# 0411tony/Yue

Hardware: AMD Instinct MI355X
Metric: BPR triplet-updates/sec at k=128 (S-round semantics, user rows sequential; the reference's exact sequential semantics: secondary.exact) (higher is better)
Workload: dtype f32

## Files before the change

### yue_amd/csrc/bpr_host.hip

```cpp
#include "host_common.hpp"

#include "train_kernels.hpp"
#include "round_kernels.hpp"

using yue_host::fail;
using yue_host::kr_of;
using yue_host::with_kr;
static_assert(yue::kNllSlots == yue_host::kNllSlotsHost && yue::kHeaderSlack == yue_host::kHeaderSlackHost &&
              yue::kMetaStageMax == (uint32_t)yue_host::kMetaStageMaxHost, "host_common.hpp mirrors these");

namespace {

yue::TrainArgs make_args(yue_ctx *c, double lr, double regU, double regI) {
    yue::TrainArgs a{};
    a.P = c->P.p; a.Q = c->Q.p; a.dP = c->dP.p; a.dQ = c->dQ.p;
    a.stage = c->Q.p ? c->Q.p + (size_t)c->n * c->k : nullptr;
    a.ev_u = c->ev_u.p; a.ev_i = c->ev_i.p; a.ev_j = c->ev_j.p;
    a.indptr = c->indptr.p; a.indices = c->indices.p;
    a.nll_slots = c->scal.p;
    a.m = c->m; a.n = c->n; a.k = c->k;
    a.lr = lr;
    a.ru = (float)(lr * regU);
    a.ri = (float)(lr * regI);
    a.neg_lo = 0; a.neg_range = (int32_t)c->n;
// ... 23 lines not shown

int tpw_of(const yue_ctx *c, bool meta) { return c->opt_round_tpw ? c->opt_round_tpw : default_round_tpw(kr_of(c->k), meta); }

constexpr int64_t kMetaRangeMax = 37 * 1024;
constexpr int64_t kMetaRangesMax = 12;
constexpr int64_t kRoundGenerationsMax = 6;
constexpr double kRoundEventsPerItemRow = 4.0;

bool meta_bucketed(const yue_ctx *c) { return c->n > kMetaRangeMax * kMetaRangesMax || c->opt_round_bucket; }
bool meta_path_fits(const yue_ctx *c) { return c->opt_round_meta && c->n <= ((int64_t)yue::kBucketRangesMax << yue::kBucketShift); }

int default_round_events(yue_ctx *c, double n_rows, int64_t *out) {
    const bool fold = yue_host::fold_path(c);
    const int tpw = tpw_of(c, fold);
    int per_cu = 0, cus = 0;
    hipError_t e = hipSuccess;
    if (!with_round_instance(kr_of(c->k), tpw, [&](auto kr, auto t) {
            e = fold ? hipOccupancyMaxActiveBlocksPerMultiprocessor(&per_cu, yue::k_round_m<kr(), t()>, 256, 0)
                     : hipOccupancyMaxActiveBlocksPerMultiprocessor(&per_cu, yue::k_round<kr(), t()>, 256, 0);
        }))
        return fail(YUE_ERR_ARG, "unsupported (k, TPW) combination");
    HIPCHK(e);
    per_cu = std::min(per_cu, fold ? 7 : 6);
    HIPCHK(hipDeviceGetAttribute(&cus, hipDeviceAttributeMultiprocessorCount, c->device));
    const double slots = (double)per_cu * (double)cus;
    int64_t w = (int64_t)(slots * 4.0 * tpw);
    w -= w % 1024;
    w = std::max<int64_t>(w, 1024);
    if (fold) {
        int64_t sets = std::min<int64_t>(kRoundGenerationsMax, std::max<int64_t>(1, (int64_t)(kRoundEventsPerItemRow * n_rows / (double)w)));
        if (2.0 * (double)(w * sets) < 2.0 * n_rows) sets = std::min<int64_t>(sets, 4);
        w *= sets;
    }
    *out = w;
    return YUE_OK;
}

int launch_round(yue_ctx *c, const yue::TrainArgs &a_in, int64_t e0, int64_t e1, int64_t n0, int64_t n1,
                 int parity, int apply_p) {
    unsigned long long *cnt[2] = {c->cnt0.p, c->cnt1.p};
    uint32_t *cntp[2] = {c->cntp0.p, c->cntp1.p};
    yue::RoundArgs ra{};
    ra.e_begin = e0; ra.e_end = e1; ra.n_begin = n0; ra.n_end = n1;
    ra.cnt_cur = cnt[parity]; ra.cnt_next = cnt[parity ^ 1]; ra.cntp_cur = cntp[parity]; ra.cntp_next = cntp[parity ^ 1];
    uint32_t *tab[2] = {c->tab0.p, c->tab1.p};
    ra.tab_cur = tab[parity]; ra.tab_next = tab[parity ^ 1]; ra.staged = c->staged ? 1 : 0;
    ra.apply_p = apply_p;
// ... 24 lines not shown
int launch_round_meta(yue_ctx *c, const yue::TrainArgs &a, const std::vector<int64_t> &bounds) {
    const int64_t R = (int64_t)bounds.size() - 1;
    const int64_t E = bounds.back();
    HIPCHK(c->meta_i.resize((size_t)E + yue::kHeaderSlack)); HIPCHK(c->meta_j.resize((size_t)E + yue::kHeaderSlack));
    HIPCHK(c->round_rows.resize((size_t)R)); HIPCHK(c->d_bounds.resize((size_t)R + 1));
    if (c->h_bounds != bounds) {
        HIPCHK(hipStreamSynchronize(c->stream));
        c->h_bounds = bounds;
        HIPCHK(hipMemcpyAsync(c->d_bounds.p, c->h_bounds.data(), (size_t)(R + 1) * sizeof(int64_t), hipMemcpyHostToDevice, c->stream));
    }
    HIPCHK(hipMemsetAsync(c->round_rows.p, 0, (size_t)R * sizeof(unsigned long long), c->stream));
    HIPCHK(c->fold.resize((size_t)(E + 4 * R + 8)));
    yue::MetaArgs ma{};
    ma.ev_i = a.ev_i; ma.ev_j = a.ev_j; ma.bounds = c->d_bounds.p; ma.R = R; ma.n = (int32_t)c->n;
    const bool bucketed = meta_bucketed(c);
    if (bucketed) {
        ma.range = 1 << yue::kBucketShift;
        ma.G = (int32_t)((c->n + ma.range - 1) >> yue::kBucketShift);
        HIPCHK(c->bk_touch.resize((size_t)(2 * E + 2))); HIPCHK(c->bk_ptr.resize((size_t)R * (ma.G + 1)));
        yue::BucketArgs ba{};
        ba.ev_i = a.ev_i; ba.ev_j = a.ev_j; ba.bounds = c->d_bounds.p; ba.R = R; ba.G = ma.G;
        ba.bk_touch = c->bk_touch.p; ba.bk_ptr = c->bk_ptr.p; ba.meta_i = c->meta_i.p; ba.meta_j = c->meta_j.p;
        int cus0 = 0;
        HIPCHK(hipDeviceGetAttribute(&cus0, hipDeviceAttributeMultiprocessorCount, c->device));
        hipLaunchKernelGGL(yue::k_round_bucket, dim3((unsigned)std::min<int64_t>(R, 2 * cus0)), dim3(1024), 0, c->stream, ba);
        ma.bk_touch = c->bk_touch.p; ma.bk_ptr = c->bk_ptr.p;
    } else {
        ma.G = (int32_t)((c->n + kMetaRangeMax - 1) / kMetaRangeMax);
        ma.range = (int32_t)((c->n + ma.G - 1) / ma.G);
    }
    ma.chunk = (ma.range + 1023) / 1024; ma.chunk |= 1;
    int64_t widest = 0;
    for (int64_t r = 0; r < R; ++r) widest = std::max(widest, bounds[(size_t)r + 1] - bounds[(size_t)r]);
    const double mean_touches = 2.0 * (double)widest / (double)std::max<int64_t>(1, c->n);
    const uint32_t stage_auto = (uint32_t)std::min<double>((double)yue::kMetaStageMax, std::max<double>((double)yue::kMetaStageDefault,
                                                         std::ceil(mean_touches * (kr_of(c->k) == 1 ? 4.0 : 2.0))));
    ma.stage_max = !c->staged ? 1u : c->opt_round_stage >= 2 ? (uint32_t)c->opt_round_stage : stage_auto;
    c->last_stage_max = (int)ma.stage_max;
    ma.meta_i = c->meta_i.p; ma.meta_j = c->meta_j.p; ma.round_rows = c->round_rows.p; ma.fold = c->fold.p;
    const size_t lds = (size_t)ma.range * sizeof(uint32_t);
    const void *kfn = bucketed ? (const void *)yue::k_round_meta<true> : (const void *)yue::k_round_meta<false>;
    HIPCHK(hipFuncSetAttribute(kfn, hipFuncAttributeMaxDynamicSharedMemorySize, (int)lds));
    int per_cu = 0, cus = 0;
    if (bucketed) { HIPCHK(hipOccupancyMaxActiveBlocksPerMultiprocessor(&per_cu, yue::k_round_meta<true>, 1024, lds)); }
    else { HIPCHK(hipOccupancyMaxActiveBlocksPerMultiprocessor(&per_cu, yue::k_round_meta<false>, 1024, lds)); }
    HIPCHK(hipDeviceGetAttribute(&cus, hipDeviceAttributeMultiprocessorCount, c->device));
    const int64_t grid = std::max<int64_t>(8, std::min<int64_t>((R * ma.G + 7) / 8 * 8, (int64_t)std::max(per_cu, 1) * cus / 8 * 8));
    if (bucketed) hipLaunchKernelGGL(yue::k_round_meta<true>, dim3((unsigned)grid), dim3(1024), lds, c->stream, ma);
    else
        hipLaunchKernelGGL(yue::k_round_meta<false>, dim3((unsigned)grid), dim3(1024), lds, c->stream, ma);
    HIPCHK(hipGetLastError());
    return YUE_OK;
}

void launch_round_fold(yue_ctx *c, const yue::TrainArgs &a, int64_t e0, int64_t e1, int64_t round_index) {
    yue::FoldArgs f{};
    f.fold = c->fold.p + yue::fold_base(e0, round_index); f.round_rows = c->round_rows.p + round_index; f.Q = a.Q; f.dQ = a.dQ; f.stage = a.stage; f.k = c->k; f.capacity = (uint32_t)((e1 - e0) & ~(int64_t)3);
    const dim3 fgrid((unsigned)std::min<int64_t>(c->opt_fold_blocks, std::max<int64_t>(1, (e1 - e0 + 15) / 16))), block(256);
    with_kr(c->k, [&](auto kr) { hipLaunchKernelGGL(yue::k_round_fold<kr()>, fgrid, block, 0, c->stream, f); });
}

int launch_round_m(yue_ctx *c, const yue::TrainArgs &a_in, int64_t e0, int64_t e1, int64_t round_index) {
    yue::RoundMArgs ra{};
    ra.e_begin = e0; ra.e_end = e1; ra.staged = c->staged ? 1 : 0;
    const int tpw = tpw_of(c, true);
    const int64_t waves = (e1 - e0 + tpw - 1) / tpw;
    const int64_t blocks = (waves + 3) / 4;
    if (blocks == 0) return YUE_OK;
    const dim3 grid((unsigned)blocks), block(256);
#ifdef YUE_STAMPS
// ... 109 lines not shown
        c->ev_triplets[c->ev_used] = bounds.back() - bounds.front();
        c->ev_launches[c->ev_used] = (int64_t)ne.size();
        c->ev_used++;
    }
    return YUE_OK;
}

void reset_round_state(yue_ctx *c) {
    (void)hipStreamSynchronize(c->stream);
    if (c->cnt0.p) (void)hipMemsetAsync(c->cnt0.p, 0, c->cnt0.n * sizeof(unsigned long long), c->stream);
    if (c->cnt1.p) (void)hipMemsetAsync(c->cnt1.p, 0, c->cnt1.n * sizeof(unsigned long long), c->stream);
    if (c->cntp0.p) (void)hipMemsetAsync(c->cntp0.p, 0, c->cntp0.n * sizeof(uint32_t), c->stream);
    if (c->cntp1.p) (void)hipMemsetAsync(c->cntp1.p, 0, c->cntp1.n * sizeof(uint32_t), c->stream);
    if (c->dP.p) (void)hipMemsetAsync(c->dP.p, 0, c->dP.n * sizeof(float), c->stream);
    if (c->dQ.p) (void)hipMemsetAsync(c->dQ.p, 0, c->dQ.n * sizeof(float), c->stream);
    (void)hipStreamSynchronize(c->stream);
}

}

namespace yue_host {
bool fold_path(const yue_ctx *c) { return meta_path_fits(c); }

int zero_scalars(yue_ctx *c) {
    HIPCHK(hipMemsetAsync(c->scal.p, 0, (yue::kNllSlots + 8) * sizeof(double), c->stream));
    return YUE_OK;
}

int read_scalars(yue_ctx *c, double *nll, double *sp, double *sq) {
    double *sc = c->scal.p + yue::kNllSlots;
    hipLaunchKernelGGL(yue::k_sum_slots, dim3(1), dim3(64), 0, c->stream, c->scal.p, yue::kNllSlots, sc);
    double h[3];
    HIPCHK(hipMemcpyAsync(h, sc, sizeof h, hipMemcpyDeviceToHost, c->stream));
    HIPCHK(hipStreamSynchronize(c->stream));
    if (nll) *nll = h[0];
    if (sp) *sp = h[1];
    if (sq) *sq = h[2];
    return YUE_OK;
}

int sumsq_async(yue_ctx *c, const double *p_slots) {
    double *sc = c->scal.p + yue::kNllSlots;
    HIPCHK(hipMemsetAsync(sc + 1, 0, 2 * sizeof(double), c->stream));
    if (p_slots) hipLaunchKernelGGL(yue::k_sum_slots, dim3(1), dim3(64), 0, c->stream, p_slots, yue::kNllSlots, sc + 1);
    else hipLaunchKernelGGL(yue::k_sumsq, dim3(2048), dim3(256), 0, c->stream, c->P.p, c->m * c->k, sc + 1);
    hipLaunchKernelGGL(yue::k_sumsq, dim3(2048), dim3(256), 0, c->stream, c->Q.p, c->n * c->k, sc + 2);
// ... 3 lines not shown
int upload_triplets(yue_ctx *c, const int32_t *u, const int32_t *i, const int32_t *j, int64_t T, bool validate) {
    for (int64_t t = 0; validate && t < T; ++t) {
        if (u[t] < 0 || u[t] >= c->m || i[t] < 0 || i[t] >= c->n || j[t] >= c->n)
            return fail(YUE_ERR_ARG, "triplet " + std::to_string(t) + " out of range");
    }
    HIPCHK(c->xu.resize((size_t)T + yue::kHeaderSlack)); HIPCHK(c->xi.resize((size_t)T + yue::kHeaderSlack)); HIPCHK(c->xj.resize((size_t)T + yue::kHeaderSlack));
    HIPCHK(hipMemcpyAsync(c->xu.p, u, T * sizeof(int32_t), hipMemcpyHostToDevice, c->stream));
    HIPCHK(hipMemcpyAsync(c->xi.p, i, T * sizeof(int32_t), hipMemcpyHostToDevice, c->stream));
    HIPCHK(hipMemcpyAsync(c->xj.p, j, T * sizeof(int32_t), hipMemcpyHostToDevice, c->stream));
    return YUE_OK;
}
int adam_apply_dense(yue_ctx *c, float *var, float *m, float *v, float *grad, int64_t count, double lr, int64_t step) {
    const double b1 = 0.9, b2 = 0.999;
    const float lr_t = (float)(lr * std::sqrt(1.0 - std::pow(b2, (double)step)) / (1.0 - std::pow(b1, (double)step)));
    hipLaunchKernelGGL(yue::k_adam, dim3((unsigned)std::min<int64_t>(8192, (count + 255) / 256)), dim3(256), 0, c->stream, var, m, v, grad, count, lr_t, 0.9f, 0.999f, 1e-8f);
    HIPCHK(hipGetLastError());
    return YUE_OK;
}
int adam_apply(yue_ctx *c, double lr, int64_t step) {
    const int rc = adam_apply_dense(c, c->P.p, c->aU_m.p, c->aU_v.p, c->dP.p, c->m * (int64_t)c->k, lr, step);
    return rc ? rc : adam_apply_dense(c, c->Q.p, c->aV_m.p, c->aV_v.p, c->dQ.p, c->n * (int64_t)c->k, lr, step);
}
}
using yue_host::zero_scalars; using yue_host::read_scalars; using yue_host::sumsq_async; using yue_host::upload_triplets;

extern "C" {

int yue_bpr_replay(yue_ctx *c, const int32_t *u, const int32_t *i, const int32_t *j, int64_t T,
                   double lr, double regU, double regI, double *nll_out) {
    if (!c || !c->have_factors) return fail(YUE_ERR_ARG, "yue_bpr_replay: no factors uploaded");
    if (T < 0 || (T > 0 && (!u || !i || !j))) return fail(YUE_ERR_ARG, "yue_bpr_replay: bad triplet arrays");
    HIPCHK(hipSetDevice(c->device));
    if (!c->opt_replay_levels) {
        int rc = upload_triplets(c, u, i, j, T, false);
        if (rc) return rc;
        if ((rc = zero_scalars(c))) return rc;
        if ((rc = yue_host::chain_stream(c, T, lr, regU, regI))) return rc;
        return read_scalars(c, nll_out, nullptr, nullptr);
    }
    std::vector<int32_t> lastP((size_t)c->m, 0), lastQ((size_t)c->n, 0), lvl((size_t)T);
    int32_t nlev = 0;
    for (int64_t t = 0; t < T; ++t) {
        if (u[t] < 0 || u[t] >= c->m || i[t] < 0 || i[t] >= c->n || j[t] >= c->n) return fail(YUE_ERR_ARG, "triplet " + std::to_string(t) + " out of range");
        if (j[t] < 0) { lvl[(size_t)t] = 0; continue; }
        if (i[t] == j[t]) return fail(YUE_ERR_ARG, "triplet " + std::to_string(t) + ": i == j");
        int32_t l = std::max(lastP[(size_t)u[t]], std::max(lastQ[(size_t)i[t]], lastQ[(size_t)j[t]])) + 1;
        lvl[(size_t)t] = l;
// ... 109 lines not shown

int yue_adam_step(yue_ctx *c, const int32_t *u, const int32_t *i, const int32_t *j, int64_t T, double lr, double reg, int64_t step, double *loss_out) {
    if (!c || !c->have_factors) return fail(YUE_ERR_ARG, "yue_adam_step: no factors uploaded");
    if (T <= 0 || !u || !i || !j || step < 1) return fail(YUE_ERR_ARG, "yue_adam_step: bad argument (T > 0, step >= 1)");
    HIPCHK(hipSetDevice(c->device));
    if (c->adam_m != c->m || c->adam_n != c->n || c->adam_k != c->k) { const int rc0 = yue_adam_reset(c); if (rc0) return rc0; }
    for (int64_t t = 0; t < T; ++t)
        if (u[t] < 0 || u[t] >= c->m || i[t] < 0 || i[t] >= c->n || j[t] < 0 || j[t] >= c->n) return fail(YUE_ERR_ARG, "yue_adam_step: triplet " + std::to_string(t) + " out of range");
    int rc = upload_triplets(c, u, i, j, T, true);
    if (rc) return rc;
    if ((rc = zero_scalars(c))) return rc;
    yue::MbArgs a{};
    a.U = c->P.p; a.V = c->Q.p; a.gU = c->dP.p; a.gV = c->dQ.p; a.k = c->k; a.u = c->xu.p; a.i = c->xi.p; a.j = c->xj.p; a.T = T;
    a.reg = (float)reg; a.loss_slots = c->scal.p;
    const dim3 grid((unsigned)(((T + 31) / 32 + 3) / 4));
    with_kr(c->k, [&](auto kr) { hipLaunchKernelGGL(yue::k_mb_grad<kr()>, grid, dim3(256), 0, c->stream, a); });
    if ((rc = yue_host::adam_apply(c, lr, step))) return rc;
    return read_scalars(c, loss_out, nullptr, nullptr);
}

int yue_sample_negatives(yue_ctx *c, uint64_t seed, uint32_t epoch, int32_t *j_out) {
    if (!c || !c->have_inter || !j_out) return fail(YUE_ERR_ARG, "yue_sample_negatives: no interactions uploaded");
    HIPCHK(hipSetDevice(c->device));
    yue::TrainArgs a = make_args(c, 0, 0, 0);
    a.seed = seed; a.epoch = epoch;
    if (c->E > 0) {
        hipLaunchKernelGGL(yue::k_sample, dim3((unsigned)((c->E + 255) / 256)), dim3(256), 0, c->stream, a, c->E);
        HIPCHK(hipGetLastError());
        HIPCHK(hipMemcpyAsync(j_out, c->ev_j.p, c->E * sizeof(int32_t), hipMemcpyDeviceToHost, c->stream));
    }
    HIPCHK(hipStreamSynchronize(c->stream));
    return YUE_OK;
}

int yue_sumsq(yue_ctx *c, double *sp, double *sq) {
    if (!c || !c->have_factors) return fail(YUE_ERR_ARG, "yue_sumsq: no factors uploaded");
    HIPCHK(hipSetDevice(c->device));
    int rc = sumsq_async(c);
    if (rc) return rc;
    double h[2];
    HIPCHK(hipMemcpyAsync(h, c->scal.p + yue::kNllSlots + 1, sizeof h, hipMemcpyDeviceToHost, c->stream));
    HIPCHK(hipStreamSynchronize(c->stream));
    if (sp) *sp = h[0];
    if (sq) *sq = h[1];
    return YUE_OK;
}

int yue_bpr_epoch(yue_ctx *c, uint64_t seed, uint32_t epoch, int64_t round_events, double lr, double regU, double regI,
                  double *nll_out, double *sumsqP_out, double *sumsqQ_out) {
    if (!c || !c->have_factors || !c->have_inter) return fail(YUE_ERR_ARG, "yue_bpr_epoch: upload factors and interactions first");
    if (round_events < 0) return fail(YUE_ERR_ARG, "yue_bpr_epoch: round_events must be positive (or 0 for the device's default)");
    HIPCHK(hipSetDevice(c->device));
    yue::TrainArgs a = make_args(c, lr, regU, regI);
    a.seed = seed + 0x632BE59BD9B4E019ull * (uint64_t)c->rank;
    a.epoch = epoch;
    int rc = zero_scalars(c);
    if (rc) return rc;
    const int64_t E = c->E;
    if (E > 0) hipLaunchKernelGGL(yue::k_sample, dim3((unsigned)((E + 255) / 256)), dim3(256), 0, c->stream, a, E);
    if (c->opt_epoch_exact) {
        if (yue_host::on_communicator(c) && c->nranks > 1) return fail(YUE_ERR_ARG, "yue_bpr_epoch: option epoch_exact runs on one GPU (the sequential order spans all item shards)");
        if ((rc = yue_host::chain_epoch(c, lr, regU, regI))) return rc;
        if ((rc = sumsq_async(c))) return rc;
        return read_scalars(c, nll_out, sumsqP_out, sumsqQ_out);
    }
    std::vector<int64_t> bounds;
    double tot[2] = {(double)E, (double)c->n};
    if (yue_host::on_communicator(c)) {
        if ((rc = yue_allreduce_f64(c, tot, 2))) return rc;
        if ((rc = zero_scalars(c))) return rc;
    }
    const double etot = tot[0];
    if (round_events == 0 && (rc = default_round_events(c, tot[1] / c->nranks, &round_events))) return rc;
    int64_t ub = 1, group = 1;
    if ((rc = yue_epoch_plan(c->m, c->k, round_events, etot, c->nranks, &ub, &group, nullptr))) return rc;
    if (!yue_host::on_communicator(c)) group = std::max<int64_t>(1, (c->m + ub - 1) / ub);
    else group = std::max<int64_t>(1, ((int64_t)c->opt_comm_group_mb << 20) / std::max<int64_t>(1, ub * c->k * 4));
    std::vector<int64_t> ublock;
    for (int64_t u0 = 0; u0 < c->m; u0 += ub) { ublock.push_back(u0); bounds.push_back(c->h_ev_ptr[(size_t)u0]); }
    ublock.push_back(c->m); bounds.push_back(E);
    const int64_t R = (int64_t)ublock.size() - 1;
    const bool seq_user = !yue_host::on_communicator(c) && c->opt_round_user_seq && meta_path_fits(c);
    if (seq_user) {
        HIPCHK(c->d_ev_ptr.resize((size_t)c->m + 1));
        if (!c->d_ev_ptr_valid) {
            HIPCHK(hipMemcpyAsync(c->d_ev_ptr.p, c->h_ev_ptr.data(), ((size_t)c->m + 1) * sizeof(int64_t), hipMemcpyHostToDevice, c->stream));
            c->d_ev_ptr_valid = true;
        }
        HIPCHK(c->margins.resize((size_t)std::max<int64_t>(E, 1)));
    }
    c->psq_in_rounds = seq_user && c->all_users_have_events && E > 0;
    if (c->psq_in_rounds) {
        HIPCHK(c->psq_slots.resize((size_t)yue::kNllSlots));
        HIPCHK(hipMemsetAsync(c->psq_slots.p, 0, (size_t)yue::kNllSlots * sizeof(double), c->stream));
    }
    c->last_round_user_seq = 0;
    auto after = [&](int64_t r) -> int {
        if (seq_user && !c->bigq) { c->last_round_user_seq = 1; return YUE_OK; }
        if ((r + 1) % group != 0 && r + 1 != R) return YUE_OK;
        const int64_t g_first = ublock[(size_t)(r - (r % group))], g_last = ublock[(size_t)r + 1];
        const int64_t first = g_first * c->k, count = (g_last - g_first) * c->k;
        const dim3 grid((unsigned)std::min<int64_t>(4096, (count + 255) / 256));
        if (!yue_host::on_communicator(c)) {
            hipLaunchKernelGGL(yue::k_apply_range, grid, dim3(256), 0, c->stream, c->P.p, c->dP.p, first, count);
            return YUE_OK;
        }
        HIPCHK(hipEventRecord(c->ev_rounds, c->stream));
        HIPCHK(hipStreamWaitEvent(c->comm_stream, c->ev_rounds, 0));
        c->comm_collectives += 1;
        c->comm_bytes += (double)count * sizeof(float);
        if (const int rcr = yue_host::reduce_user_block(c, first, count, c->comm_stream)) return rcr;
        hipLaunchKernelGGL(yue::k_apply_range, grid, dim3(256), 0, c->comm_stream, c->P.p, c->dP.p, first, count);
        return YUE_OK;
// ... 88 lines not shown
```

### yue_amd/csrc/chain_host.hip

```cpp
#include "host_common.hpp"

#include <rocprim/rocprim.hpp>

#include "chain_kernels.hpp"

using yue_host::fail;
using yue_host::kr_of;

namespace {

int bits_for(uint64_t values) { int b = 1; while ((1ull << b) < values) ++b; return b; }

int rank_in_stream(yue_ctx *c, DevBuf<uint32_t> &key, DevBuf<uint32_t> &val, int64_t count, uint32_t nkeys, uint32_t *ord_a, uint32_t *ord_b) {
    if (count == 0) return YUE_OK;
    HIPCHK(c->ch_key2.resize((size_t)count)); HIPCHK(c->ch_val2.resize((size_t)count)); HIPCHK(c->ch_seg.resize((size_t)nkeys + 1));
    rocprim::double_buffer<uint32_t> dk(key.p, c->ch_key2.p), dv(val.p, c->ch_val2.p);
    size_t tmp = 0;
    const unsigned end_bit = (unsigned)bits_for((uint64_t)nkeys + 1);
    HIPCHK(rocprim::radix_sort_pairs(nullptr, tmp, dk, dv, (size_t)count, 0u, end_bit, c->stream));
    HIPCHK(c->ch_tmp.resize(tmp + 16));
    HIPCHK(rocprim::radix_sort_pairs(c->ch_tmp.p, tmp, dk, dv, (size_t)count, 0u, end_bit, c->stream));
    const dim3 grid((unsigned)((count + 255) / 256));
    hipLaunchKernelGGL(yue::k_chain_seg, grid, dim3(256), 0, c->stream, dk.current(), count, nkeys, c->ch_seg.p);
    hipLaunchKernelGGL(yue::k_chain_ord, grid, dim3(256), 0, c->stream, dk.current(), dv.current(), count, nkeys, c->ch_seg.p, ord_a, ord_b);
// ... 100 lines not shown
        unsigned long long h[8];
        HIPCHK(hipMemcpy(h, c->ch_stats.p, sizeof h, hipMemcpyDeviceToHost));
        if (split)
            fprintf(stderr, "[chain3 stats] per triplet: wave C %.0f cycles of work + %.0f waiting for a packet; wave L %.0f cycles per step without a wait (%llu steps) and %.0f waiting for room in the ring; wave S %.0f cycles waiting for packets or answers (%llu triplets)\n",
                    h[1] ? (double)h[0] / h[1] : 0.0, h[1] ? (double)h[2] / h[1] : 0.0, h[4] ? (double)h[3] / h[4] : 0.0, h[4], h[1] ? (double)h[7] / h[1] : 0.0, h[6] ? (double)h[5] / h[6] : 0.0, h[6]);
        else
        fprintf(stderr, "[chain stats] steps without a wait: %llu, %.0f cycles each; steps that waited: %llu (%.2f %%), %.0f cycles each; per run outside the steps: %.0f cycles (%llu runs)\n",
                h[1], h[1] ? (double)h[0] / h[1] : 0.0, h[3], 100.0 * h[3] / (double)(h[1] + h[3] + 1e-9), h[3] ? (double)h[2] / h[3] : 0.0, h[5] ? (double)h[4] / h[5] : 0.0, h[5]);
    }
#endif
    c->chain_runs = R; c->chain_waves = (one_xcd ? c->chain_groups : blocks) * waves_per_block;
    { float ms = 0.0f; HIPCHK(hipEventElapsedTime(&ms, c->ev_chain0, c->ev_chain1)); c->chain_kernel_us = (int64_t)(1e3 * ms); }
    if (st) return fail(YUE_ERR_HIP, std::string("exact path: a wave gave up waiting for a row (") + ((st & 2u) ? "a row's version ran past a waiting touch" : "spin limit") +
                                    "): internal error, the factors on the device are not usable");
    return YUE_OK;
}

}

namespace yue_host {

int chain_epoch(yue_ctx *c, double lr, double regU, double regI) {
    if (c->E == 0) return YUE_OK;
    HIPCHK(c->d_ev_ptr.resize((size_t)c->m + 1));
    if (!c->d_ev_ptr_valid) {
        HIPCHK(hipMemcpyAsync(c->d_ev_ptr.p, c->h_ev_ptr.data(), ((size_t)c->m + 1) * sizeof(int64_t), hipMemcpyHostToDevice, c->stream));
        c->d_ev_ptr_valid = true;
    }
    return chain_launch(c, nullptr, c->ev_i.p, c->ev_j.p, c->E, c->d_ev_ptr.p, nullptr, nullptr, c->m, lr, regU, regI);
}

int chain_stream(yue_ctx *c, int64_t T, double lr, double regU, double regI) {
    if (T == 0) return YUE_OK;
    if (T >= (1ll << 31)) return fail(YUE_ERR_ARG, "exact path: at most 2^31 - 1 triplets per call");
    HIPCHK(c->ch_head.resize((size_t)T)); HIPCHK(c->ch_incl.resize((size_t)T));
    const dim3 tgrid((unsigned)((T + 255) / 256));
    hipLaunchKernelGGL(yue::k_chain_heads, tgrid, dim3(256), 0, c->stream, c->xu.p, T, c->ch_head.p);
    size_t tmp = 0;
    HIPCHK(rocprim::inclusive_scan(nullptr, tmp, c->ch_head.p, c->ch_incl.p, (size_t)T, rocprim::plus<uint32_t>(), c->stream));
    HIPCHK(c->ch_tmp.resize(tmp + 16));
    HIPCHK(rocprim::inclusive_scan(c->ch_tmp.p, tmp, c->ch_head.p, c->ch_incl.p, (size_t)T, rocprim::plus<uint32_t>(), c->stream));
    uint32_t R32 = 0;
    HIPCHK(hipMemcpyAsync(&R32, c->ch_incl.p + (T - 1), sizeof R32, hipMemcpyDeviceToHost, c->stream));
    HIPCHK(hipStreamSynchronize(c->stream));
    const int64_t R = R32;
    HIPCHK(c->ch_run_ptr.resize((size_t)R + 1)); HIPCHK(c->ch_run_u.resize((size_t)R)); HIPCHK(c->ch_ord_u.resize((size_t)R));
    HIPCHK(c->ch_rkey.resize((size_t)R)); HIPCHK(c->ch_rval.resize((size_t)R));
    hipLaunchKernelGGL(yue::k_chain_runs, tgrid, dim3(256), 0, c->stream, c->xu.p, c->ch_head.p, c->ch_incl.p, T, c->ch_run_ptr.p, c->ch_run_u.p, c->ch_rkey.p, c->ch_rval.p, (uint32_t)c->m);
    int rc = rank_in_stream(c, c->ch_rkey, c->ch_rval, R, (uint32_t)c->m, c->ch_ord_u.p, nullptr);
    if (rc) return rc;
    return chain_launch(c, c->xu.p, c->xi.p, c->xj.p, T, c->ch_run_ptr.p, c->ch_run_u.p, c->ch_ord_u.p, R, lr, regU, regI);
// ... 4 lines not shown
```

### yue_amd/csrc/core_host.hip

```cpp
#include "host_common.hpp"

namespace yue_host {
thread_local std::string g_err;
int fail(int code, const std::string &msg) { g_err = msg; return code; }
}
using yue_host::fail;
void yue_comm_release(yue_ctx *c);

extern "C" {

const char *yue_last_error(void) { return yue_host::g_err.c_str(); }
int yue_version(void) { return 1; }

int yue_ctx_create(int device, yue_ctx **out) {
    if (!out) return fail(YUE_ERR_ARG, "yue_ctx_create: out is NULL");
    int ndev = 0;
    HIPCHK(hipGetDeviceCount(&ndev));
    if (ndev <= 0) return fail(YUE_ERR_HIP, "no HIP device visible: libyue_hip needs an MI355X (no CPU fallback exists)");
    if (device < 0 || device >= ndev) return fail(YUE_ERR_ARG, "device ordinal out of range");
    HIPCHK(hipSetDevice(device));
    yue_ctx *c = new yue_ctx();
    c->device = device;
    const auto init = [c]() -> int {
        HIPCHK(hipStreamCreateWithFlags(&c->stream, hipStreamNonBlocking));
// ... 109 lines not shown
        if (indptr[u + 1] < indptr[u] || ev_ptr[u + 1] < ev_ptr[u]) return fail(YUE_ERR_ARG, "yue_set_interactions: offsets must be non-decreasing");
        for (int64_t t = indptr[u]; t < indptr[u + 1]; ++t) {
            if (indices[t] < 0 || indices[t] >= n) return fail(YUE_ERR_ARG, "yue_set_interactions: item id out of range");
            if (t > indptr[u] && indices[t] <= indices[t - 1]) return fail(YUE_ERR_ARG, "yue_set_interactions: rows must be sorted and unique");
        }
        if (indptr[u + 1] - indptr[u] >= n) return fail(YUE_ERR_ARG, "yue_set_interactions: a user listened to every item (the reference's sampler would never return, BPR.py:47)");
    }
    const int64_t nnz = indptr[m], E = ev_ptr[m];
    {
        int64_t prev = -1, max_gap = 0;
        for (int64_t u = 0; u < m; ++u) if (ev_ptr[u + 1] > ev_ptr[u]) { if (prev >= 0) max_gap = std::max(max_gap, u - prev); prev = u; }
        if (max_gap * c->k * 4 >= (1ll << 31)) return fail(YUE_ERR_ARG, "yue_set_interactions: more than 2 GiB of user-factor rows between two consecutive users with events");
    }
    std::vector<int32_t> evu((size_t)E);
    for (int64_t u = 0; u < m; ++u)
        for (int64_t e = ev_ptr[u]; e < ev_ptr[u + 1]; ++e) {
            if (ev_i[e] < 0 || ev_i[e] >= n) return fail(YUE_ERR_ARG, "yue_set_interactions: event item out of range");
            evu[(size_t)e] = (int32_t)u;
        }
    c->E = E; c->nnz = nnz;
    c->h_ev_ptr.assign(ev_ptr, ev_ptr + m + 1);
    c->all_users_have_events = true;
    for (int64_t u = 0; u < m; ++u) if (ev_ptr[u + 1] <= ev_ptr[u]) { c->all_users_have_events = false; break; }
    c->d_ev_ptr_valid = false;
    HIPCHK(c->indptr.resize(m + 1)); HIPCHK(c->indices.resize(std::max<int64_t>(nnz, 1)));
    HIPCHK(c->ev_u.resize((size_t)E + yue_host::kHeaderSlackHost)); HIPCHK(c->ev_i.resize((size_t)E + yue_host::kHeaderSlackHost)); HIPCHK(c->ev_j.resize((size_t)E + yue_host::kHeaderSlackHost));
    HIPCHK(hipMemcpyAsync(c->indptr.p, indptr, (m + 1) * sizeof(int64_t), hipMemcpyHostToDevice, c->stream));
    HIPCHK(hipMemcpyAsync(c->indices.p, indices, nnz * sizeof(int32_t), hipMemcpyHostToDevice, c->stream));
    HIPCHK(hipMemcpyAsync(c->ev_u.p, evu.data(), E * sizeof(int32_t), hipMemcpyHostToDevice, c->stream));
    HIPCHK(hipMemcpyAsync(c->ev_i.p, ev_i, E * sizeof(int32_t), hipMemcpyHostToDevice, c->stream));
    HIPCHK(hipStreamSynchronize(c->stream));
    c->have_inter = true;
    return YUE_OK;
}


}
```

### yue_amd/csrc/host_common.hpp

```cpp
#pragma once
#include "../../include/yue_hip.h"

#include <hip/hip_runtime.h>

#include <algorithm>
#include <cmath>
#include <cstdio>
#include <cstdlib>
#include <cstring>
#include <string>
#include <type_traits>
#include <vector>

struct ncclComm;
struct yue_wrmf;
struct yue_knn;
struct yue_expo;
struct yue_cof;
struct yue_cnet;
struct yue_s2v;
struct yue_lgcn;
struct yue_ngcf;
struct yue_ipf;

// ... 38 lines not shown
    }
}

}

using yue_host::DevBuf;

struct yue_ctx {
    int device = 0;
    hipStream_t stream = nullptr;
    int64_t m = 0, n = 0, E = 0, nnz = 0;
    int k = 0;
    bool have_factors = false, have_inter = false;
    DevBuf<float> P, Q, dP, dQ;
    DevBuf<float> margins;
    DevBuf<double> psq_slots;
    DevBuf<unsigned long long> cnt0, cnt1;
    DevBuf<uint32_t> cntp0, cntp1;
    DevBuf<uint32_t> tab0, tab1;
    bool staged = false;
    bool bigq = false;
    DevBuf<uint32_t> meta_i, meta_j;
    DevBuf<unsigned long long> round_rows;
    DevBuf<uint2> fold, bk_touch;
    DevBuf<uint32_t> bk_ptr;
    DevBuf<int64_t> d_bounds;
    std::vector<int64_t> h_bounds;
#ifdef YUE_STAMPS
    DevBuf<unsigned long long> stamps;
    int64_t stamp_launch = -1, update_launches = 0, stamp_waves = 0;
#endif
    DevBuf<int32_t> ev_u, ev_i, ev_j, indices;
    DevBuf<int64_t> indptr;
    DevBuf<int32_t> xu, xi, xj, xk;
    DevBuf<double> x_loss;
    DevBuf<float> aU_m, aU_v, aV_m, aV_v;
    int64_t adam_m = 0, adam_n = 0; int adam_k = 0;
    DevBuf<double> scal;
    std::vector<int64_t> h_ev_ptr;
    bool all_users_have_events = false;
    bool psq_in_rounds = false;
    DevBuf<int32_t> s_users, s_ids, s_mask_idx, s_flags;
    DevBuf<int32_t> s_few, s_few_ids;
    DevBuf<float> s_few_scores;
    int64_t scan_few_users = 0;
    DevBuf<int64_t> s_mask_ptr;
// ... 6 lines not shown
    int opt_scan_two_phase = 1;
    int64_t opt_scan_streams_min_users = 262144;
    int opt_scan_slabs = 4;
    int opt_scan_streams = 2;
    int opt_scan_filter_ub = 3;
    int opt_scan_growth = 0;
    int scan_chunks = 0;
    int scan_used_bf16 = 0;
    int opt_scan_f32 = 0;
    int opt_scan_batch = 0;
    int opt_round_tpw = 0;
    int opt_topn_true = 0;
    int scan_settle = 0;
    int last_stage_max = 0;
    int opt_round_stage = 1;
    int opt_round_bucket = 0;
    int opt_fold_blocks = 1536;
    int opt_round_user_seq = 1;
    int opt_round_fast = 1;
    int last_round_user_seq = 0;
    int opt_comm_group_mb = 8;
    int opt_round_cus_reserved = 0;
    int64_t comm_compute_waits = 0;
    int opt_round_meta = 1;
    int timing_stride = 0;
    std::vector<std::pair<hipEvent_t, hipEvent_t>> ev_pool;
    std::vector<int64_t> ev_triplets, ev_launches;
    size_t ev_used = 0;
    DevBuf<double> fP, fBi, f_coef, f_x, f_hist, f_scores, f_out_sc;
    DevBuf<float> fQ;
    DevBuf<int64_t> f_ptr;
    DevBuf<int32_t> f_items, f_negs, f_ids, f_flags;
    DevBuf<int64_t> f_uq_ptr, f_neg_ptr;
    DevBuf<int32_t> f_uq_items, f_loc_i, f_loc_j;
    DevBuf<float> f_wq, f_dQ;
    DevBuf<double> f_wp, f_wb, f_dP, f_dB;
    DevBuf<unsigned> f_cnt;
    int64_t fn = 0;
    int fk = 0;
    int opt_fism_inplace = 1;
    int opt_fism_lds = 1;
    DevBuf<uint32_t> ch_key, ch_val, ch_key2, ch_val2, ch_seg, ch_ord_i, ch_ord_j, ch_head, ch_incl, ch_ord_u, ch_rkey, ch_rval;
    DevBuf<int64_t> ch_run_ptr, d_ev_ptr;
    DevBuf<int32_t> ch_run_u;
    DevBuf<unsigned char> ch_tmp;
    DevBuf<unsigned> ch_Qv, ch_Pv;
    DevBuf<unsigned long long> ch_ctl;
    DevBuf<unsigned long long> ch_stats;
    bool d_ev_ptr_valid = false;
    int opt_epoch_exact = 0;
    int opt_replay_levels = 0;
    int opt_chain_split = -1;
    int opt_chain_ring = 0;
    int opt_chain_xcd = 0;
    int opt_chain_fast = 0;
    int opt_chain_waves = 0;
    int64_t opt_chain_spin = 0;
    int64_t chain_runs = 0, chain_waves = 0, chain_groups = 0, chain_kernel_us = 0, replay_levels = 0;
    hipEvent_t ev_chain0 = nullptr, ev_chain1 = nullptr;
    ncclComm *comm = nullptr;
    int rank = 0, nranks = 1;
    hipStream_t comm_stream = nullptr;
    hipEvent_t ev_rounds = nullptr, ev_comm = nullptr;
    hipEvent_t ev_t_rounds = nullptr, ev_t_comm = nullptr;
    int (*seam_reduce)(void *host, int64_t count, int dtype, void *user) = nullptr;
    void *seam_user = nullptr;
    std::vector<float> seam_buf;
    int64_t comm_collectives = 0;
    double comm_bytes = 0.0, comm_wait_ms = 0.0;
    int comm_version = 0, comm_nranks_reported = 0;
    hipEvent_t ev_scan0 = nullptr, ev_scan1 = nullptr;
    yue_wrmf *wrmf = nullptr;
    yue_knn *knn = nullptr;
    yue_ipf *ipf = nullptr;
    yue_expo *expo = nullptr;
    yue_cof *cof = nullptr;
    yue_cnet *cnet = nullptr;
    yue_s2v *s2v = nullptr;
    yue_lgcn *lgcn = nullptr;
    int64_t opt_lgcn_hub = 1024;
    int64_t lgcn_hubs = 0, lgcn_parts = 0;
    int64_t lgcn_ns[4] = {0, 0, 0, 0};
    yue_ngcf *ngcf = nullptr;
    int64_t opt_ngcf_hub = 1024;
    int64_t ngcf_hubs = 0, ngcf_parts = 0;
    int64_t ngcf_ns[6] = {0, 0, 0, 0, 0, 0};
};

namespace yue_host {
inline bool on_communicator(const yue_ctx *c) { return c->comm != nullptr || c->seam_reduce != nullptr; }
bool fold_path(const yue_ctx *c);
int zero_scalars(yue_ctx *c);
int read_scalars(yue_ctx *c, double *nll, double *sp, double *sq);
int sumsq_async(yue_ctx *c, const double *p_slots = nullptr);
int upload_triplets(yue_ctx *c, const int32_t *u, const int32_t *i, const int32_t *j, int64_t T, bool validate);
int adam_apply(yue_ctx *c, double lr, int64_t step);
int adam_apply_dense(yue_ctx *c, float *var, float *m, float *v, float *grad, int64_t count, double lr, int64_t step);
int reduce_user_block(yue_ctx *c, int64_t first, int64_t count, hipStream_t stream);
int chain_epoch(yue_ctx *c, double lr, double regU, double regI);
int chain_stream(yue_ctx *c, int64_t T, double lr, double regU, double regI);
void wrmf_release(yue_ctx *c);
int wrmf_set_option(yue_ctx *c, const std::string &key, int64_t value);
int wrmf_get_option(yue_ctx *c, const std::string &key, int64_t *value);
struct WrmfPairsView {
    const int64_t *ptr, *cptr, *cbeg, *cend;
    const int32_t *idx, *cnt, *sched, *cpos;
    int64_t rows, n_long, chunks, n_nonempty;
    int64_t generation;
};
bool wrmf_pairs_view(const yue_ctx *c, int side, WrmfPairsView *v);
int wrmf_gram(yue_ctx *c, int side, const double **G);
void knn_release(yue_ctx *c);
int knn_set_option(yue_ctx *c, const std::string &key, int64_t value);
int knn_get_option(yue_ctx *c, const std::string &key, int64_t *value);
void ipf_release(yue_ctx *c);
int ipf_set_option(yue_ctx *c, const std::string &key, int64_t value);
int ipf_get_option(yue_ctx *c, const std::string &key, int64_t *value);
// ... 16 lines not shown
```

### yue_amd/csrc/options_host.hip

```cpp
#include "host_common.hpp"

#include <limits>

using yue_host::fail;

namespace {

struct Option {
    const char *name;
    int64_t (*get)(yue_ctx *);
    void (*put)(yue_ctx *, int64_t);
    int (*set)(const Option &, yue_ctx *, int64_t);
    int64_t lo, hi;
    const char *refusal;
    std::vector<int64_t> also;
};
#define YUE_AT(member) [](yue_ctx *c) -> int64_t { return c->member; }, [](yue_ctx *c, int64_t v) { c->member = (decltype(c->member))v; }

int set_flag(const Option &o, yue_ctx *c, int64_t value) { o.put(c, value != 0); return YUE_OK; }

int set_ranged(const Option &o, yue_ctx *c, int64_t value) {
    if ((value < o.lo || value > o.hi) && std::find(o.also.begin(), o.also.end(), value) == o.also.end())
        return fail(YUE_ERR_ARG, std::string("yue_set_option: ") + o.name + " " + o.refusal);
    o.put(c, value);
// ... 31 lines not shown

#ifdef YUE_STAMPS
int set_stamp_launch(const Option &, yue_ctx *c, int64_t value) { c->stamp_launch = value; c->update_launches = 0; return YUE_OK; }
#endif

const Option kOptions[] = {
    {"scan_f32", YUE_AT(opt_scan_f32), set_flag},
    {"scan_batch", YUE_AT(opt_scan_batch), set_ranged, 0, 1, "must be 0 or 1"},
    {"scan_two_phase", YUE_AT(opt_scan_two_phase), set_flag},
    {"scan_growth", YUE_AT(opt_scan_growth), set_ranged, 2, 64, "must be 0 (automatic) or 2..64", {0}},
    {"scan_filter_ub", YUE_AT(opt_scan_filter_ub), set_ranged, 1, 3, "must be 1, 2 or 3"},
    {"scan_streams", YUE_AT(opt_scan_streams), set_ranged, 1, 2, "must be 1 or 2"},
    {"scan_slabs", YUE_AT(opt_scan_slabs), set_ranged, 2, 64, "must be 2..64"},
    {"scan_streams_min_users", YUE_AT(opt_scan_streams_min_users), set_ranged, 1024, std::numeric_limits<int64_t>::max(), "must be at least 1024"},
    {"scan_last_chunks", YUE_AT(scan_chunks)},
    {"scan_last_few_users", YUE_AT(scan_few_users)},
    {"scan_last_settle", YUE_AT(scan_settle)},
    {"topn_true", YUE_AT(opt_topn_true), set_flag},
    {"fism_lds", YUE_AT(opt_fism_lds), set_flag},
    {"fism_inplace", YUE_AT(opt_fism_inplace), set_flag},
    {"round_stage", YUE_AT(opt_round_stage), set_ranged, 0, yue_host::kMetaStageMaxHost, "must be 0, 1 or 2..64"},
    {"round_last_stage_max", YUE_AT(last_stage_max)},
    {"round_meta", YUE_AT(opt_round_meta), set_flag},
    {"comm_group_mb", YUE_AT(opt_comm_group_mb), set_ranged, 1, 4096, "must be 1..4096"},
    {"round_cus_reserved", YUE_AT(opt_round_cus_reserved), set_round_cus_reserved},
    {"comm_last_compute_waits", YUE_AT(comm_compute_waits)},
    {"round_user_seq", YUE_AT(opt_round_user_seq), set_flag},
    {"round_fast", YUE_AT(opt_round_fast), set_flag},
    {"round_last_user_seq", YUE_AT(last_round_user_seq)},
    {"round_bucket", YUE_AT(opt_round_bucket), set_flag},
    {"fold_blocks", YUE_AT(opt_fold_blocks), set_ranged, 1, 65536, "out of range"},
    {"round_tpw", YUE_AT(opt_round_tpw), set_round_tpw},
    {"round_path", round_path},
#ifdef YUE_STAMPS
    {"debug_stamp_launch", nullptr, nullptr, set_stamp_launch},
#endif
    {"epoch_exact", YUE_AT(opt_epoch_exact), set_flag},
    {"replay_levels", YUE_AT(opt_replay_levels), set_flag},
    {"chain_waves", YUE_AT(opt_chain_waves), set_ranged, 0, 8, "must be 0..8"},
    {"chain_split", YUE_AT(opt_chain_split), set_ranged, -1, 1, "must be -1, 0 or 1"},
    {"chain_fast", YUE_AT(opt_chain_fast), set_flag},
    {"chain_xcd", YUE_AT(opt_chain_xcd), set_flag},
    {"chain_ring", YUE_AT(opt_chain_ring), set_ranged, 0, 0, "must be 0, 8 or 16", {8, 16}},
    {"chain_spin", YUE_AT(opt_chain_spin), set_ranged, 0, 0x7fffffff, "out of range"},
    {"chain_last_us", YUE_AT(chain_kernel_us)},
    {"chain_last_runs", YUE_AT(chain_runs)},
// ... 62 lines not shown
```

### yue_amd/csrc/train_kernels.hpp

```cpp
#pragma once
#include "bpr_device.hpp"

namespace yue {

__global__ void __launch_bounds__(256) k_sample(TrainArgs a, int64_t E) {
    int64_t e = (int64_t)blockIdx.x * blockDim.x + threadIdx.x;
    if (e < E) a.ev_j[e] = sample_negative(a, a.ev_u[e], e);
}

template <int KR>
__global__ void __launch_bounds__(256) k_bpr_level(TrainArgs a, int64_t e_begin, int64_t e_end, int tpw) {
    const int lane = threadIdx.x & 63;
    const int64_t wave = (int64_t)blockIdx.x * (blockDim.x >> 6) + (threadIdx.x >> 6);
    const int64_t base = e_begin + wave * tpw;
    if (base >= e_end) return;
    const int cnt = (int)((e_end - base) < (int64_t)tpw ? (e_end - base) : (int64_t)tpw);
    int u = 0, i = 0, j = 0;
    if (lane < cnt) { u = a.ev_u[base + lane]; i = a.ev_i[base + lane]; j = a.ev_j[base + lane]; }
    const int k = a.k;
    double nll = 0.0;
    for (int t = 0; t < cnt; ++t) {
        const int64_t tu = __builtin_amdgcn_readlane(u, t);
        const int64_t ti = __builtin_amdgcn_readlane(i, t);
        const int64_t tj = __builtin_amdgcn_readlane(j, t);
        float p[KR], qi[KR], qj[KR];
#pragma unroll
        for (int r = 0; r < KR; ++r) {
            const int e = 64 * r + lane;
            p[r] = e < k ? a.P[tu * k + e] : 0.0f;
            qi[r] = e < k ? a.Q[ti * k + e] : 0.0f;
// ... 482 lines not shown
```

Baseline: 1.844 billion.

## Add per-user wave negative sampler and cache device attribute queries

Adds a new negative-sampling kernel that assigns a wavefront to each user. The user's positive row is loaded into lanes once, and membership of each candidate draw is tested with a cross-lane binary search (ds_bpermute), replacing per-event scans of the row. It is enabled by default when there are enough events per user. The change also caches the CU count and the meta-kernel occupancy and LDS attribute setup across calls, and uploads the event pointer array once at interaction upload instead of lazily each epoch. The binary search assumes each user's positive indices are sorted, and it must match the old sampler's rejection semantics (same ctr_draw attempts), otherwise the sampled negatives would change.

```diff
diff --git a/yue_amd/csrc/bpr_host.hip b/yue_amd/csrc/bpr_host.hip
--- a/yue_amd/csrc/bpr_host.hip
+++ b/yue_amd/csrc/bpr_host.hip
@@ -69,7 +69,7 @@
         return fail(YUE_ERR_ARG, "unsupported (k, TPW) combination");
     HIPCHK(e);
     per_cu = std::min(per_cu, fold ? 7 : 6);
-    HIPCHK(hipDeviceGetAttribute(&cus, hipDeviceAttributeMultiprocessorCount, c->device));
+    if (const int rc = yue_host::device_cus(c, &cus)) return rc;
     const double slots = (double)per_cu * (double)cus;
     int64_t w = (int64_t)(slots * 4.0 * tpw);
     w -= w % 1024;
@@ -140,7 +140,7 @@
         ba.ev_i = a.ev_i; ba.ev_j = a.ev_j; ba.bounds = c->d_bounds.p; ba.R = R; ba.G = ma.G;
         ba.bk_touch = c->bk_touch.p; ba.bk_ptr = c->bk_ptr.p; ba.meta_i = c->meta_i.p; ba.meta_j = c->meta_j.p;
         int cus0 = 0;
-        HIPCHK(hipDeviceGetAttribute(&cus0, hipDeviceAttributeMultiprocessorCount, c->device));
+        if (const int rc = yue_host::device_cus(c, &cus0)) return rc;
         hipLaunchKernelGGL(yue::k_round_bucket, dim3((unsigned)std::min<int64_t>(R, 2 * cus0)), dim3(1024), 0, c->stream, ba);
         ma.bk_touch = c->bk_touch.p; ma.bk_ptr = c->bk_ptr.p;
     } else {
@@ -157,13 +157,17 @@
     c->last_stage_max = (int)ma.stage_max;
     ma.meta_i = c->meta_i.p; ma.meta_j = c->meta_j.p; ma.round_rows = c->round_rows.p; ma.fold = c->fold.p;
     const size_t lds = (size_t)ma.range * sizeof(uint32_t);
-    const void *kfn = bucketed ? (const void *)yue::k_round_meta<true> : (const void *)yue::k_round_meta<false>;
-    HIPCHK(hipFuncSetAttribute(kfn, hipFuncAttributeMaxDynamicSharedMemorySize, (int)lds));
-    int per_cu = 0, cus = 0;
-    if (bucketed) { HIPCHK(hipOccupancyMaxActiveBlocksPerMultiprocessor(&per_cu, yue::k_round_meta<true>, 1024, lds)); }
-    else { HIPCHK(hipOccupancyMaxActiveBlocksPerMultiprocessor(&per_cu, yue::k_round_meta<false>, 1024, lds)); }
-    HIPCHK(hipDeviceGetAttribute(&cus, hipDeviceAttributeMultiprocessorCount, c->device));
-    const int64_t grid = std::max<int64_t>(8, std::min<int64_t>((R * ma.G + 7) / 8 * 8, (int64_t)std::max(per_cu, 1) * cus / 8 * 8));
+    if (c->meta_resident == 0 || c->meta_lds != lds || c->meta_lds_bucketed != bucketed) {
+        const void *kfn = bucketed ? (const void *)yue::k_round_meta<true> : (const void *)yue::k_round_meta<false>;
+        const size_t lds_max = (size_t)(bucketed ? (int64_t)1 << yue::kBucketShift : kMetaRangeMax) * sizeof(uint32_t);
+        HIPCHK(hipFuncSetAttribute(kfn, hipFuncAttributeMaxDynamicSharedMemorySize, (int)lds_max));
+        int per_cu = 0, cus = 0;
+        if (bucketed) { HIPCHK(hipOccupancyMaxActiveBlocksPerMultiprocessor(&per_cu, yue::k_round_meta<true>, 1024, lds)); }
+        else { HIPCHK(hipOccupancyMaxActiveBlocksPerMultiprocessor(&per_cu, yue::k_round_meta<false>, 1024, lds)); }
+        if (const int rc = yue_host::device_cus(c, &cus)) return rc;
+        c->meta_resident = std::max(per_cu, 1) * cus; c->meta_lds = lds; c->meta_lds_bucketed = bucketed;
+    }
+    const int64_t grid = std::max<int64_t>(8, std::min<int64_t>((R * ma.G + 7) / 8 * 8, (int64_t)c->meta_resident / 8 * 8));
     if (bucketed) hipLaunchKernelGGL(yue::k_round_meta<true>, dim3((unsigned)grid), dim3(1024), lds, c->stream, ma);
     else
         hipLaunchKernelGGL(yue::k_round_meta<false>, dim3((unsigned)grid), dim3(1024), lds, c->stream, ma);
@@ -319,6 +323,31 @@
 namespace yue_host {
 bool fold_path(const yue_ctx *c) { return meta_path_fits(c); }
 
+int device_cus(yue_ctx *c, int *cus) {
+    if (c->cus == 0) HIPCHK(hipDeviceGetAttribute(&c->cus, hipDeviceAttributeMultiprocessorCount, c->device));
+    *cus = c->cus;
+    return YUE_OK;
+}
+
+int sample_async(yue_ctx *c, uint64_t seed, uint32_t epoch) {
+    if (c->E == 0) return YUE_OK;
+    yue::TrainArgs a = make_args(c, 0, 0, 0);
+    a.seed = seed; a.epoch = epoch;
+    c->last_sample_users = c->opt_sample_users && c->E >= 32 * c->m;
+    if (!c->last_sample_users) {
+        hipLaunchKernelGGL(yue::k_sample, dim3((unsigned)((c->E + 255) / 256)), dim3(256), 0, c->stream, a, c->E);
+        return YUE_OK;
+    }
+    int cus = 0;
+    if (const int rc = device_cus(c, &cus)) return rc;
+    const int64_t waves = c->opt_sample_blocks ? 4 * (int64_t)c->opt_sample_blocks : 32 * (int64_t)cus;
+    const int per_wave = (int)std::min<int64_t>(64, std::max<int64_t>(4, (c->m + 4 * waves - 1) / (4 * waves) * 4));
+    const int64_t groups = (c->m + per_wave - 1) / per_wave;
+    const int64_t blocks = c->opt_sample_blocks ? std::min<int64_t>(c->opt_sample_blocks, (groups + 3) / 4) : (groups + 3) / 4;
+    hipLaunchKernelGGL(yue::k_sample_users, dim3((unsigned)blocks), dim3(256), 0, c->stream, a, c->d_ev_ptr.p, c->indptr.p, c->indices.p, c->ev_j.p, per_wave);
+    return YUE_OK;
+}
+
 int zero_scalars(yue_ctx *c) {
     HIPCHK(hipMemsetAsync(c->scal.p, 0, (yue::kNllSlots + 8) * sizeof(double), c->stream));
     return YUE_OK;
@@ -368,7 +397,7 @@
     return rc ? rc : adam_apply_dense(c, c->Q.p, c->aV_m.p, c->aV_v.p, c->dQ.p, c->n * (int64_t)c->k, lr, step);
 }
 }
-using yue_host::zero_scalars; using yue_host::read_scalars; using yue_host::sumsq_async; using yue_host::upload_triplets;
+using yue_host::sample_async; using yue_host::zero_scalars; using yue_host::read_scalars; using yue_host::sumsq_async; using yue_host::upload_triplets;
 
 extern "C" {
 
@@ -524,10 +553,8 @@
 int yue_sample_negatives(yue_ctx *c, uint64_t seed, uint32_t epoch, int32_t *j_out) {
     if (!c || !c->have_inter || !j_out) return fail(YUE_ERR_ARG, "yue_sample_negatives: no interactions uploaded");
     HIPCHK(hipSetDevice(c->device));
-    yue::TrainArgs a = make_args(c, 0, 0, 0);
-    a.seed = seed; a.epoch = epoch;
+    if (const int rc = sample_async(c, seed, epoch)) return rc;
     if (c->E > 0) {
-        hipLaunchKernelGGL(yue::k_sample, dim3((unsigned)((c->E + 255) / 256)), dim3(256), 0, c->stream, a, c->E);
         HIPCHK(hipGetLastError());
         HIPCHK(hipMemcpyAsync(j_out, c->ev_j.p, c->E * sizeof(int32_t), hipMemcpyDeviceToHost, c->stream));
     }
@@ -559,7 +586,7 @@
     int rc = zero_scalars(c);
     if (rc) return rc;
     const int64_t E = c->E;
-    if (E > 0) hipLaunchKernelGGL(yue::k_sample, dim3((unsigned)((E + 255) / 256)), dim3(256), 0, c->stream, a, E);
+    if ((rc = sample_async(c, a.seed, epoch))) return rc;
     if (c->opt_epoch_exact) {
         if (yue_host::on_communicator(c) && c->nranks > 1) return fail(YUE_ERR_ARG, "yue_bpr_epoch: option epoch_exact runs on one GPU (the sequential order spans all item shards)");
         if ((rc = yue_host::chain_epoch(c, lr, regU, regI))) return rc;
@@ -583,14 +610,7 @@
     ublock.push_back(c->m); bounds.push_back(E);
     const int64_t R = (int64_t)ublock.size() - 1;
     const bool seq_user = !yue_host::on_communicator(c) && c->opt_round_user_seq && meta_path_fits(c);
-    if (seq_user) {
-        HIPCHK(c->d_ev_ptr.resize((size_t)c->m + 1));
-        if (!c->d_ev_ptr_valid) {
-            HIPCHK(hipMemcpyAsync(c->d_ev_ptr.p, c->h_ev_ptr.data(), ((size_t)c->m + 1) * sizeof(int64_t), hipMemcpyHostToDevice, c->stream));
-            c->d_ev_ptr_valid = true;
-        }
-        HIPCHK(c->margins.resize((size_t)std::max<int64_t>(E, 1)));
-    }
+    if (seq_user) HIPCHK(c->margins.resize((size_t)std::max<int64_t>(E, 1)));
     c->psq_in_rounds = seq_user && c->all_users_have_events && E > 0;
     if (c->psq_in_rounds) {
         HIPCHK(c->psq_slots.resize((size_t)yue::kNllSlots));
diff --git a/yue_amd/csrc/chain_host.hip b/yue_amd/csrc/chain_host.hip
--- a/yue_amd/csrc/chain_host.hip
+++ b/yue_amd/csrc/chain_host.hip
@@ -146,11 +146,6 @@
 
 int chain_epoch(yue_ctx *c, double lr, double regU, double regI) {
     if (c->E == 0) return YUE_OK;
-    HIPCHK(c->d_ev_ptr.resize((size_t)c->m + 1));
-    if (!c->d_ev_ptr_valid) {
-        HIPCHK(hipMemcpyAsync(c->d_ev_ptr.p, c->h_ev_ptr.data(), ((size_t)c->m + 1) * sizeof(int64_t), hipMemcpyHostToDevice, c->stream));
-        c->d_ev_ptr_valid = true;
-    }
     return chain_launch(c, nullptr, c->ev_i.p, c->ev_j.p, c->E, c->d_ev_ptr.p, nullptr, nullptr, c->m, lr, regU, regI);
 }
 
diff --git a/yue_amd/csrc/core_host.hip b/yue_amd/csrc/core_host.hip
--- a/yue_amd/csrc/core_host.hip
+++ b/yue_amd/csrc/core_host.hip
@@ -155,11 +155,11 @@
     c->h_ev_ptr.assign(ev_ptr, ev_ptr + m + 1);
     c->all_users_have_events = true;
     for (int64_t u = 0; u < m; ++u) if (ev_ptr[u + 1] <= ev_ptr[u]) { c->all_users_have_events = false; break; }
-    c->d_ev_ptr_valid = false;
-    HIPCHK(c->indptr.resize(m + 1)); HIPCHK(c->indices.resize(std::max<int64_t>(nnz, 1)));
+    HIPCHK(c->indptr.resize(m + 1)); HIPCHK(c->d_ev_ptr.resize((size_t)m + 1)); HIPCHK(c->indices.resize(std::max<int64_t>(nnz, 1)));
     HIPCHK(c->ev_u.resize((size_t)E + yue_host::kHeaderSlackHost)); HIPCHK(c->ev_i.resize((size_t)E + yue_host::kHeaderSlackHost)); HIPCHK(c->ev_j.resize((size_t)E + yue_host::kHeaderSlackHost));
     HIPCHK(hipMemcpyAsync(c->indptr.p, indptr, (m + 1) * sizeof(int64_t), hipMemcpyHostToDevice, c->stream));
     HIPCHK(hipMemcpyAsync(c->indices.p, indices, nnz * sizeof(int32_t), hipMemcpyHostToDevice, c->stream));
+    HIPCHK(hipMemcpyAsync(c->d_ev_ptr.p, ev_ptr, (m + 1) * sizeof(int64_t), hipMemcpyHostToDevice, c->stream));
     HIPCHK(hipMemcpyAsync(c->ev_u.p, evu.data(), E * sizeof(int32_t), hipMemcpyHostToDevice, c->stream));
     HIPCHK(hipMemcpyAsync(c->ev_i.p, ev_i, E * sizeof(int32_t), hipMemcpyHostToDevice, c->stream));
     HIPCHK(hipStreamSynchronize(c->stream));
diff --git a/yue_amd/csrc/host_common.hpp b/yue_amd/csrc/host_common.hpp
--- a/yue_amd/csrc/host_common.hpp
+++ b/yue_amd/csrc/host_common.hpp
@@ -84,6 +84,9 @@
     bool bigq = false;
     DevBuf<uint32_t> meta_i, meta_j;
     DevBuf<unsigned long long> round_rows;
+    size_t meta_lds = 0;
+    bool meta_lds_bucketed = false;
+    int meta_resident = 0, cus = 0;
     DevBuf<uint2> fold, bk_touch;
     DevBuf<uint32_t> bk_ptr;
     DevBuf<int64_t> d_bounds;
@@ -136,6 +139,9 @@
     int opt_comm_group_mb = 8;
     int opt_round_cus_reserved = 0;
     int64_t comm_compute_waits = 0;
+    int opt_sample_users = 1;
+    int opt_sample_blocks = 0;
+    int last_sample_users = 0;
     int opt_round_meta = 1;
     int timing_stride = 0;
     std::vector<std::pair<hipEvent_t, hipEvent_t>> ev_pool;
@@ -161,7 +167,6 @@
     DevBuf<unsigned> ch_Qv, ch_Pv;
     DevBuf<unsigned long long> ch_ctl;
     DevBuf<unsigned long long> ch_stats;
-    bool d_ev_ptr_valid = false;
     int opt_epoch_exact = 0;
     int opt_replay_levels = 0;
     int opt_chain_split = -1;
@@ -207,6 +212,8 @@
 int zero_scalars(yue_ctx *c);
 int read_scalars(yue_ctx *c, double *nll, double *sp, double *sq);
 int sumsq_async(yue_ctx *c, const double *p_slots = nullptr);
+int sample_async(yue_ctx *c, uint64_t seed, uint32_t epoch);
+int device_cus(yue_ctx *c, int *cus);
 int upload_triplets(yue_ctx *c, const int32_t *u, const int32_t *i, const int32_t *j, int64_t T, bool validate);
 int adam_apply(yue_ctx *c, double lr, int64_t step);
 int adam_apply_dense(yue_ctx *c, float *var, float *m, float *v, float *grad, int64_t count, double lr, int64_t step);
diff --git a/yue_amd/csrc/options_host.hip b/yue_amd/csrc/options_host.hip
--- a/yue_amd/csrc/options_host.hip
+++ b/yue_amd/csrc/options_host.hip
@@ -77,6 +77,9 @@
     {"round_stage", YUE_AT(opt_round_stage), set_ranged, 0, yue_host::kMetaStageMaxHost, "must be 0, 1 or 2..64"},
     {"round_last_stage_max", YUE_AT(last_stage_max)},
     {"round_meta", YUE_AT(opt_round_meta), set_flag},
+    {"sample_users", YUE_AT(opt_sample_users), set_flag},
+    {"sample_blocks", YUE_AT(opt_sample_blocks), set_ranged, 0, 65536, "must be 0 (automatic) or 1..65536"},
+    {"sample_last_users", YUE_AT(last_sample_users)},
     {"comm_group_mb", YUE_AT(opt_comm_group_mb), set_ranged, 1, 4096, "must be 1..4096"},
     {"round_cus_reserved", YUE_AT(opt_round_cus_reserved), set_round_cus_reserved},
     {"comm_last_compute_waits", YUE_AT(comm_compute_waits)},
diff --git a/yue_amd/csrc/train_kernels.hpp b/yue_amd/csrc/train_kernels.hpp
--- a/yue_amd/csrc/train_kernels.hpp
+++ b/yue_amd/csrc/train_kernels.hpp
@@ -6,6 +6,80 @@
 __global__ void __launch_bounds__(256) k_sample(TrainArgs a, int64_t E) {
     int64_t e = (int64_t)blockIdx.x * blockDim.x + threadIdx.x;
     if (e < E) a.ev_j[e] = sample_negative(a, a.ev_u[e], e);
+}
+
+constexpr int32_t kNoEntry = 0x7fffffff;
+constexpr int kSampleBatch = 4;
+
+__device__ __forceinline__ bool chunk_contains(int32_t v, int32_t x) {
+    int pos = 0;
+#pragma unroll
+    for (int s = 32; s >= 1; s >>= 1) {
+        const int32_t t = __builtin_amdgcn_ds_bpermute((pos + s - 1) << 2, v);
+        pos += t < x ? s : 0;
+    }
+    return __builtin_amdgcn_ds_bpermute(pos << 2, v) == x;
+}
+
+__device__ __forceinline__ int64_t rdlane64(int64_t v, int l) {
+    const uint32_t lo = (uint32_t)__builtin_amdgcn_readlane((int)(uint32_t)v, l), hi = (uint32_t)__builtin_amdgcn_readlane((int)(uint32_t)((uint64_t)v >> 32), l);
+    return (int64_t)(((uint64_t)hi << 32) | lo);
+}
+
+__global__ void __launch_bounds__(256) k_sample_users(TrainArgs a, const int64_t *__restrict__ ev_ptr, const int64_t *__restrict__ indptr,
+                                                      const int32_t *__restrict__ indices, int32_t *__restrict__ ev_j, int per_wave) {
+    const int lane = threadIdx.x & 63;
+    const int64_t groups = (a.m + per_wave - 1) / per_wave, stride = (int64_t)gridDim.x * 4;
+    for (int64_t g = (int64_t)blockIdx.x * 4 + __builtin_amdgcn_readfirstlane((int)(threadIdx.x >> 6)); g < groups; g += stride) {
+        const int64_t mine = g * per_wave + lane, safe = mine < a.m ? mine : a.m - 1;
+        const bool there = lane < per_wave && mine < a.m;
+        const int64_t ge0 = ev_ptr[safe], ge1 = there ? ev_ptr[safe + 1] : ge0;
+        const int64_t gr0 = indptr[safe], gr1 = there ? indptr[safe + 1] : gr0;
+        const int users = (int)(a.m - g * per_wave < per_wave ? a.m - g * per_wave : per_wave);
+        for (int b = 0; b < users; b += kSampleBatch) {
+            int64_t e0[kSampleBatch], e1[kSampleBatch], r0[kSampleBatch], r1[kSampleBatch];
+            int32_t row[kSampleBatch];
+#pragma unroll
+            for (int q = 0; q < kSampleBatch; ++q) {
+                const int t = b + q < 64 ? b + q : 63;
+                e0[q] = rdlane64(ge0, t); e1[q] = b + q < 64 ? rdlane64(ge1, t) : e0[q];
+                r0[q] = rdlane64(gr0, t); r1[q] = e1[q] > e0[q] ? rdlane64(gr1, t) : r0[q];
+                row[q] = r0[q] + lane < r1[q] ? indices[r0[q] + lane] : kNoEntry;
+            }
+            int32_t first[kSampleBatch];
+            bool hit[kSampleBatch];
+#pragma unroll
+            for (int q = 0; q < kSampleBatch; ++q) {
+                first[q] = ctr_draw(a.seed, a.epoch, (uint64_t)(e0[q] + lane), 0u, a.neg_lo, a.neg_range);
+                hit[q] = chunk_contains(row[q], first[q]);
+            }
+#pragma unroll
+            for (int q = 0; q < kSampleBatch; ++q) {
+                const int64_t row_len = r1[q] - r0[q];
+                if (e1[q] - e0[q] <= 64 && row_len <= 64 && !__ballot(hit[q] && e0[q] + lane < e1[q])) {
+                    if (e0[q] + lane < e1[q]) ev_j[e0[q] + lane] = first[q];
+                    continue;
+                }
+                for (int64_t seg = e0[q]; seg < e1[q]; seg += 64) {
+                    const int64_t e = seg + lane;
+                    uint32_t attempt = 0;
+                    int32_t cand = ctr_draw(a.seed, a.epoch, (uint64_t)e, 0u, a.neg_lo, a.neg_range), out = -1;
+                    bool pending = e < e1[q];
+                    while (__ballot(pending)) {
+                        bool in_row = chunk_contains(row[q], cand);
+                        for (int64_t c = 64; c < row_len; c += 64)
+                            in_row |= chunk_contains(r0[q] + c + lane < r1[q] ? indices[r0[q] + c + lane] : kNoEntry, cand);
+                        if (pending && !in_row) { out = cand; pending = false; }
+                        if (pending) {
+                            if (++attempt == (uint32_t)kMaxAttempts) pending = false;
+                            else cand = ctr_draw(a.seed, a.epoch, (uint64_t)e, attempt, a.neg_lo, a.neg_range);
+                        }
+                    }
+                    if (e < e1[q]) ev_j[e] = out;
+                }
+            }
+        }
+    }
 }
 
 template <int KR>
```

Result: no change. 1.862 billion (median of 6 runs) (+1.0%).
